# RoyAPTX4869/RaLD

Measured on AMD Instinct MI355X. Metric: denoising steps/sec (whole node), higher is better.
Workload: dtype bf16

## Files before the change

### rald_amd/csrc/gemm.hip

```cpp
#include <algorithm>
#include <cstdlib>
#include <type_traits>

#include "common.h"
#include "kernels.h"
#include "gemm_epilogue.h"
#include "gemm_tile.h"

namespace rald {

template <int MT, int NT, int EPI>
__device__ __forceinline__ void gemm_epilogue(f32x4 (&acc)[MT][NT], const GemmArgs& a, int mb, int nb, int64_t coff, int fr, int fq) {
    if constexpr (EPI == EPI_GEGLU) {
        bf16* C = reinterpret_cast<bf16*>(a.C) + coff;
#pragma unroll
        for (int i = 0; i < MT; ++i) {
            const int m = mb + i * 16 + fr;
            if (m >= a.M) continue;
#pragma unroll
            for (int p = 0; p < NT / 2; ++p) {
                const int nx = nb + 32 * p + 4 * fq;
                const int ng = nx + 16;
                float4 bx = *reinterpret_cast<const float4*>(a.bias + nx);
                float4 bg = *reinterpret_cast<const float4*>(a.bias + ng);
                f32x4 x = acc[i][2 * p], g = acc[i][2 * p + 1];
                bf16x4 o = pack4((x[0] + bx.x) * gelu_erf(g[0] + bg.x), (x[1] + bx.y) * gelu_erf(g[1] + bg.y),
                                 (x[2] + bx.z) * gelu_erf(g[2] + bg.z), (x[3] + bx.w) * gelu_erf(g[3] + bg.w));
                const int c = nb / 2 + 16 * p + 4 * fq;
                *reinterpret_cast<bf16x4*>(C + (int64_t)m * a.ldc + c) = o;
            }
        }
    } else {
#pragma unroll
        for (int i = 0; i < MT; ++i) {
            const int m = mb + i * 16 + fr;
            if (m >= a.M) continue;
#pragma unroll
            for (int j = 0; j < NT; ++j) {
                const int n = nb + j * 16 + 4 * fq;
                if (n >= a.N) continue;
                f32x4 v = acc[i][j];
                float4 b = make_float4(0.f, 0.f, 0.f, 0.f);
                if (a.bias) b = *reinterpret_cast<const float4*>(a.bias + n);
                const float al = n < a.alpha_ncols ? a.alpha : 1.0f;
                if constexpr (EPI == EPI_BF16) {
                    bf16* C = reinterpret_cast<bf16*>(a.C) + coff;
                    *reinterpret_cast<bf16x4*>(C + (int64_t)m * a.ldc + n) =
                        pack4(al * v[0] + b.x, al * v[1] + b.y, al * v[2] + b.z, al * v[3] + b.w);
                } else if constexpr (EPI == EPI_F32) {
                    float* C = reinterpret_cast<float*>(a.C) + coff;
                    *reinterpret_cast<float4*>(C + (int64_t)m * a.ldc + n) =
                        make_float4(al * v[0] + b.x, al * v[1] + b.y, al * v[2] + b.z, al * v[3] + b.w);
                } else {
                    float* C = reinterpret_cast<float*>(a.C) + coff;
                    float4* p = reinterpret_cast<float4*>(C + (int64_t)m * a.ldc + n);
                    float4 r = *p;
                    *p = make_float4(r.x + v[0] + b.x, r.y + v[1] + b.y, r.z + v[2] + b.z, r.w + v[3] + b.w);
                }
            }
        }
    }
}


template <int BM, int BN, int EPI>
__global__ __launch_bounds__(256) void gemm_nt_kernel(GemmArgs a) {
    constexpr int BK = 64;
    constexpr int MT = BM / 32;
    constexpr int NT = BN / 32;
    constexpr int PA = BM / 32;
    constexpr int PB = BN / 32;
    __shared__ __attribute__((aligned(16))) unsigned char smem[2 * (BM + BN) * BK * 2];
    bf16x8* sA = reinterpret_cast<bf16x8*>(smem);
    bf16x8* sB = reinterpret_cast<bf16x8*>(smem + 2 * BM * BK * 2);

    const int tid = threadIdx.x;
    const int lane = tid & 63;
    const int wave = tid >> 6;
    const int wm = wave >> 1, wn = wave & 1;
    const int m0 = blockIdx.y * BM, n0 = blockIdx.x * BN;
    int64_t oa, ob, coff;
    gemm_batch_offsets(a, blockIdx.z, oa, ob, coff);
    const bf16* A = a.A + oa;
    const bf16* B = a.B + ob;

    const int srow = tid >> 3, schunk = tid & 7;
    const bf16* gA[PA];
    const bf16* gB[PB];
#pragma unroll
    for (int p = 0; p < PA; ++p) {
        int r = m0 + srow + 32 * p;
        r = r < a.M ? r : a.M - 1;
        gA[p] = A + (int64_t)r * a.lda + schunk * 8;
    }
#pragma unroll
    for (int p = 0; p < PB; ++p) {
        int r = n0 + srow + 32 * p;
        r = r < a.N ? r : a.N - 1;
        gB[p] = B + (int64_t)r * a.ldb + schunk * 8;
    }
    bf16x8 rA[PA], rB[PB];
    auto load_tile = [&](int kt) {
#pragma unroll
        for (int p = 0; p < PA; ++p) rA[p] = *reinterpret_cast<const bf16x8*>(gA[p] + kt * BK);
#pragma unroll
        for (int p = 0; p < PB; ++p) rB[p] = *reinterpret_cast<const bf16x8*>(gB[p] + kt * BK);
    };
    auto store_tile = [&](int buf) {
#pragma unroll
        for (int p = 0; p < PA; ++p) {
            int r = srow + 32 * p;
            sA[(buf * BM + r) * 8 + RALD_SWZ(r, schunk)] = rA[p];
        }
#pragma unroll
        for (int p = 0; p < PB; ++p) {
            int r = srow + 32 * p;
            sB[(buf * BN + r) * 8 + RALD_SWZ(r, schunk)] = rB[p];
        }
    };

    f32x4 acc[MT][NT];
#pragma unroll
    for (int i = 0; i < MT; ++i)
#pragma unroll
        for (int j = 0; j < NT; ++j) acc[i][j] = f32x4{0.f, 0.f, 0.f, 0.f};

    const int nk = a.K / BK;
    load_tile(0);
    store_tile(0);
    __syncthreads();
    const int fr = lane & 15, fq = lane >> 4;
    for (int kt = 0; kt < nk; ++kt) {
        const int buf = kt & 1;
        if (kt + 1 < nk) load_tile(kt + 1);
#pragma unroll
        for (int kk = 0; kk < 2; ++kk) {
            bf16x8 fa[MT], fb[NT];
            const int chunk = kk * 4 + fq;
#pragma unroll
            for (int i = 0; i < MT; ++i) {
                int r = wm * (BM / 2) + i * 16 + fr;
                fa[i] = sA[(buf * BM + r) * 8 + RALD_SWZ(r, chunk)];
            }
#pragma unroll
            for (int j = 0; j < NT; ++j) {
                int r = wn * (BN / 2) + j * 16 + fr;
                fb[j] = sB[(buf * BN + r) * 8 + RALD_SWZ(r, chunk)];
            }
#pragma unroll
            for (int i = 0; i < MT; ++i)
#pragma unroll
                for (int j = 0; j < NT; ++j)
                    acc[i][j] = __builtin_amdgcn_mfma_f32_16x16x32_bf16(fb[j], fa[i], acc[i][j], 0, 0, 0);
        }
        if (kt + 1 < nk) store_tile(buf ^ 1);
        __syncthreads();
    }
    gemm_epilogue<MT, NT, EPI>(acc, a, m0 + wm * (BM / 2), n0 + wn * (BN / 2), coff, fr, fq);
}

template <int BM, int BN, int WM, int WN, int NSTAGE, int EPI>
__global__ __launch_bounds__(WM * WN * 64) void gemm_nt_glds_kernel(GemmArgs a) {
    constexpr int BK = 64;
    constexpr int WAVES = WM * WN;
    constexpr int MT = BM / (16 * WM);
    constexpr int NT = BN / (16 * WN);
    constexpr int CA = BM / 8 / WAVES;
    constexpr int CB = BN / 8 / WAVES;
    constexpr int STAGE_BYTES = (BM + BN) * BK * 2;
    extern __shared__ __attribute__((aligned(16))) unsigned char smem[];

    const int tid = threadIdx.x;
    const int lane = tid & 63;
    const int wave = __builtin_amdgcn_readfirstlane(tid >> 6);
    const int wm = wave / WN, wn = wave % WN;
    int tm, tn;
    xcd_strip_tile(tm, tn);
    const int ntn = gridDim.x, nt = ntn * gridDim.y;
    int bz = blockIdx.z;
    if (nt < 8 && (gridDim.z & 7) == 0) {
        const int g = (blockIdx.z * gridDim.y + blockIdx.y) * gridDim.x + blockIdx.x;
        const int slot = g >> 3;
        bz = (slot / nt) * 8 + (g & 7);
        const int tl = slot % nt;
        tm = tl / ntn;
        tn = tl % ntn;
    }
    const int m0 = tm * BM, n0 = tn * BN;
    int64_t oa, ob, coff;
    gemm_batch_offsets(a, bz, oa, ob, coff);
    const bf16* A = a.A + oa;
    const bf16* B = a.B + ob;

    const int nk = a.K / BK;
    const bf16* gA[CA];
    const bf16* gB[CB];
    dma_sources<WAVES>(gA, A, a.lda, m0, a.M, wave, lane);
    dma_sources<WAVES>(gB, B, a.ldb, n0, a.N, wave, lane);
    auto stage = [&](int kt, int buf) { dma_stage<BM, WAVES>(gA, gB, kt, nk, smem + buf * STAGE_BYTES, wave); };

    f32x4 acc[MT][NT];
#pragma unroll
    for (int i = 0; i < MT; ++i)
#pragma unroll
        for (int j = 0; j < NT; ++j) acc[i][j] = f32x4{0.f, 0.f, 0.f, 0.f};

    const int fr = lane & 15, fq = lane >> 4;
    auto read_frags = [&](int buf, int kk, bf16x8 (&fa)[MT], bf16x8 (&fb)[NT]) {
        const bf16x8* sA = reinterpret_cast<const bf16x8*>(smem + buf * STAGE_BYTES);
        const bf16x8* sB = sA + BM * 8;
        const int chunk = kk * 4 + fq;
#pragma unroll
        for (int i = 0; i < MT; ++i) {
            const int r = wm * (BM / WM) + i * 16 + fr;
            fa[i] = sA[r * 8 + RALD_SWZ(r, chunk)];
        }
#pragma unroll
        for (int j = 0; j < NT; ++j) {
            const int r = wn * (BN / WN) + j * 16 + fr;
            fb[j] = sB[r * 8 + RALD_SWZ(r, chunk)];
        }
    };
    auto mfma_all = [&](const bf16x8 (&fa)[MT], const bf16x8 (&fb)[NT]) {
#pragma unroll
        for (int i = 0; i < MT; ++i)
#pragma unroll
            for (int j = 0; j < NT; ++j)
                acc[i][j] = __builtin_amdgcn_mfma_f32_16x16x32_bf16(fb[j], fa[i], acc[i][j], 0, 0, 0);
    };
    if constexpr (NSTAGE == 2) {
        bf16x8 fa0[MT], fb0[NT], fa1[MT], fb1[NT];
        constexpr int W_ALL = 0x0070;
        constexpr int W_ST1 = ((CA + CB) & 15) | (((CA + CB) >> 4) << 14) | 0x0f70;
        stage(0, 0);
        if (nk > 1) { stage(1, 1); __builtin_amdgcn_s_waitcnt(W_ST1); }
        else __builtin_amdgcn_s_waitcnt(W_ALL);
        __builtin_amdgcn_s_barrier();
        read_frags(0, 0, fa0, fb0);
        read_frags(0, 1, fa1, fb1);
        mfma_all(fa0, fb0);
        __builtin_amdgcn_s_waitcnt(W_ALL);
        __builtin_amdgcn_s_barrier();
        auto body = [&](int kt, auto with_dma) {
            const int cur = kt & 1;
            if constexpr (decltype(with_dma)::value) stage(kt + 1, cur ^ 1);
            read_frags(cur, 0, fa0, fb0);
            mfma_all(fa1, fb1);
            if constexpr (MT + NT == 12 && MT * NT == 32) {
                if constexpr (decltype(with_dma)::value) {
#pragma unroll
                    for (int g = 0; g < CA + CB; ++g) {
                        __builtin_amdgcn_sched_group_barrier(0x008, 1, 0);
                        __builtin_amdgcn_sched_group_barrier(0x010, 1, 0);
                    }
#pragma unroll
                    for (int g = 0; g < 12; ++g) {
                        __builtin_amdgcn_sched_group_barrier(0x008, 2, 0);
                        __builtin_amdgcn_sched_group_barrier(0x100, 1, 0);
                    }
                } else {
#pragma unroll
                    for (int g = 0; g < 12; ++g) {
                        __builtin_amdgcn_sched_group_barrier(0x008, 2, 0);
                        __builtin_amdgcn_sched_group_barrier(0x100, 1, 0);
                    }
                    __builtin_amdgcn_sched_group_barrier(0x008, 8, 0);
                }
            }
            __builtin_amdgcn_sched_barrier(0);
            read_frags(cur, 1, fa1, fb1);
            mfma_all(fa0, fb0);
            if constexpr (MT + NT == 12 && MT * NT == 32) {
#pragma unroll
                for (int g = 0; g < 12; ++g) {
                    __builtin_amdgcn_sched_group_barrier(0x008, 2, 0);
                    __builtin_amdgcn_sched_group_barrier(0x100, 1, 0);
                }
                __builtin_amdgcn_sched_group_barrier(0x008, 8, 0);
            }
            __builtin_amdgcn_sched_barrier(0);
            __builtin_amdgcn_s_waitcnt(W_ALL);
            __builtin_amdgcn_s_barrier();
        };
        for (int kt = 1; kt + 1 < nk; ++kt) body(kt, std::true_type{});
        if (nk > 1) body(nk - 1, std::false_type{});
        mfma_all(fa1, fb1);
    } else {
#pragma unroll
        for (int s = 0; s < NSTAGE - 1; ++s)
            if (s < nk) stage(s, s);
        for (int kt = 0; kt < nk; ++kt) {
            if (kt + NSTAGE - 2 < nk) asm volatile("s_waitcnt vmcnt(%0)" ::"n"((NSTAGE - 2) * (CA + CB)) : "memory");
            else asm volatile("s_waitcnt vmcnt(0)" ::: "memory");
            asm volatile("" ::: "memory");
            __builtin_amdgcn_s_barrier();
            asm volatile("" ::: "memory");
            if (kt + NSTAGE - 1 < nk) stage(kt + NSTAGE - 1, (kt + NSTAGE - 1) % NSTAGE);
#pragma unroll
            for (int kk = 0; kk < 2; ++kk) {
                bf16x8 fa[MT], fb[NT];
                read_frags(kt % NSTAGE, kk, fa, fb);
                mfma_all(fa, fb);
            }
        }
    }
    if constexpr (NSTAGE != 2) {
        asm volatile("" ::: "memory");
        __builtin_amdgcn_s_barrier();
        asm volatile("" ::: "memory");
    }
    gemm_epilogue_lds<MT, NT, EPI>(acc, a, m0 + wm * (BM / WM), n0 + wn * (BN / WN), coff, lane, smem + wave * EPI_PATCH_BYTES,
                                   reinterpret_cast<float*>(smem + WAVES * EPI_PATCH_BYTES) + wave * NT * 16);
}

constexpr int PERSIST_LDS_BYTES = 160 * 1024;
__device__ __forceinline__ void batched_tile_at(int g, int ntn, int ntm, int nbatch, int& bz, int& tm, int& tn) {
    const int nt = ntn * ntm;
    if (nt < 8 && (nbatch & 7) == 0) {
        const int slot = g >> 3;
        bz = (slot / nt) * 8 + (g & 7);
        const int tl = slot % nt;
        tm = tl / ntn;
        tn = tl % ntn;
    } else {
        bz = g / nt;
        xcd_strip_tile_at(g - bz * nt, ntn, ntm, tm, tn);
    }
}
template <int EPI>
__global__ __launch_bounds__(512) void gemm_nt_persist_kernel(GemmArgs a) {
    static_assert(EPI == EPI_BF16 || EPI == EPI_GEGLU || EPI == EPI_SOFTMAX64, "the persistent engine is built for the three bf16-output epilogues");
    constexpr bool BATCHED = EPI == EPI_SOFTMAX64, BIAS = EPI != EPI_SOFTMAX64;
    constexpr int BM = 256, BN = 256, BK = 64, WN = 2, MT = 4, NT = 8;
    constexpr int DW = 4;
    constexpr int CP = BM / 8 / DW;
    constexpr int STAGE_BYTES = (BM + BN) * BK * 2;
    constexpr int OC = (EPI == EPI_GEGLU) ? NT * 8 : NT * 16;
    constexpr int ROWB = OC * 2, STRIDE = ROWB + 16, LPR = ROWB / 16;
    constexpr int PR = (EPI == EPI_GEGLU) ? 16 : 8;
    constexpr int PATCH = PR * STRIDE;
    constexpr int NSLOT = 12;
    constexpr int RPI = 64 / LPR;
    constexpr int BIAS_OFF = 2 * STAGE_BYTES + 31 * 1024;
    static_assert(2 * STAGE_BYTES + NSLOT * PATCH <= BIAS_OFF && BIAS_OFF + BN * 4 <= PERSIST_LDS_BYTES && PR % RPI == 0 && (MT * 16 / PR) % 2 == 0,
                  "LDS plan; an even number of steps per tile keeps the slot parity across tiles");
    extern __shared__ __attribute__((aligned(16))) unsigned char smem[];
    float* tbias = reinterpret_cast<float*>(smem + BIAS_OFF);

    const int tid = threadIdx.x;
    const int lane = tid & 63;
    const int wave = __builtin_amdgcn_readfirstlane(tid >> 6);
    const int wm = wave / WN, wn = wave % WN;
    const bool dma = wave < DW;
    const int ntm = a.M / BM, ntn = a.N / BN, nt = ntm * ntn * (BATCHED ? a.batch : 1);
    const int nk = a.K / BK;
    const int fr = lane & 15, fq = lane >> 4;

    const unsigned voA = (unsigned)((lane >> 3) * (int)a.lda + RALD_SWZ(lane >> 3, lane & 7) * 8) * 2u;
    const unsigned voB = (unsigned)((lane >> 3) * (int)a.ldb + RALD_SWZ(lane >> 3, lane & 7) * 8) * 2u;
    const unsigned lds0 = (unsigned)(uintptr_t)(lds_void*)smem;
    auto dma_piece = [&](const char* base, unsigned voff, unsigned lds) {
        asm volatile("s_nop 0\n\tglobal_load_lds_dwordx4 %0, %1" ::"v"(voff), "s"(base), "{m0}"(lds) : "memory");
    };
    struct Tile { int64_t oa, ob, oc; int m0, n0; };
    auto tile_at = [&](int t) {
        int bz = 0, tm, tn;
        if constexpr (BATCHED) batched_tile_at(t, ntn, ntm, a.batch, bz, tm, tn);
        else xcd_strip_tile_at(t, ntn, ntm, tm, tn);
        return Tile{bz * a.strideA, bz * a.strideB, bz * a.strideC, tm * BM, tn * BN};
    };
    auto stage = [&](const Tile& T, int kt, int buf) {
        const char* pa = reinterpret_cast<const char*>(a.A) + (T.oa + (int64_t)(T.m0 + 8 * wave) * a.lda + kt * BK) * 2;
        const char* pb = reinterpret_cast<const char*>(a.B) + (T.ob + (int64_t)(T.n0 + 8 * wave) * a.ldb + kt * BK) * 2;
        const unsigned s = lds0 + buf * STAGE_BYTES + wave * 1024;
#pragma unroll
        for (int p = 0; p < CP; ++p) dma_piece(pa + (int64_t)p * (8 * DW * 2) * a.lda, voA, s + p * DW * 1024);
#pragma unroll
        for (int p = 0; p < CP; ++p) dma_piece(pb + (int64_t)p * (8 * DW * 2) * a.ldb, voB, s + BM * 128 + p * DW * 1024);
    };
    auto read_frags = [&](int buf, int kk, bf16x8 (&fa)[MT], bf16x8 (&fb)[NT]) {
        const bf16x8* sA = reinterpret_cast<const bf16x8*>(smem + buf * STAGE_BYTES);
        const bf16x8* sB = sA + BM * 8;
        const int chunk = kk * 4 + fq;
#pragma unroll
        for (int i = 0; i < MT; ++i) {
            const int r = wm * (MT * 16) + i * 16 + fr;
            fa[i] = sA[r * 8 + RALD_SWZ(r, chunk)];
        }
#pragma unroll
        for (int j = 0; j < NT; ++j) {
            const int r = wn * (NT * 16) + j * 16 + fr;
            fb[j] = sB[r * 8 + RALD_SWZ(r, chunk)];
        }
    };
    f32x4 acc[MT][NT];
    auto mfma_all = [&](const bf16x8 (&fa)[MT], const bf16x8 (&fb)[NT]) {
#pragma unroll
        for (int i = 0; i < MT; ++i)
#pragma unroll
            for (int j = 0; j < NT; ++j)
                acc[i][j] = __builtin_amdgcn_mfma_f32_16x16x32_bf16(fb[j], fa[i], acc[i][j], 0, 0, 0);
    };
    constexpr int W_ALL = 0x0070;
    constexpr int W_LGKM = 0xc07f;
    constexpr int W_ST1 = ((2 * CP) & 15) | (((2 * CP) >> 4) << 14) | 0x0070;
    auto hand_over = [&]() {
        if (dma) __builtin_amdgcn_s_waitcnt(W_ALL);
        else __builtin_amdgcn_s_waitcnt(W_LGKM);
        __builtin_amdgcn_s_barrier();
    };
    bf16x8 fa0[MT], fb0[NT], fa1[MT], fb1[NT];
    auto body = [&](const Tile& T, int kt, bool with_dma) {
        const int cur = kt & 1;
        if (with_dma && dma) stage(T, kt + 1, cur ^ 1);
        __builtin_amdgcn_sched_barrier(0);
        read_frags(cur, 0, fa0, fb0);
        mfma_all(fa1, fb1);
#pragma unroll
        for (int g = 0; g < 12; ++g) {
            __builtin_amdgcn_sched_group_barrier(0x008, 2, 0);
            __builtin_amdgcn_sched_group_barrier(0x100, 1, 0);
        }
        __builtin_amdgcn_sched_group_barrier(0x008, 8, 0);
        __builtin_amdgcn_sched_barrier(0);
        read_frags(cur, 1, fa1, fb1);
        mfma_all(fa0, fb0);
#pragma unroll
        for (int g = 0; g < 12; ++g) {
            __builtin_amdgcn_sched_group_barrier(0x008, 2, 0);
            __builtin_amdgcn_sched_group_barrier(0x100, 1, 0);
        }
        __builtin_amdgcn_sched_group_barrier(0x008, 8, 0);
        __builtin_amdgcn_sched_barrier(0);
        hand_over();
    };

    if constexpr (BIAS)
        if (!a.bias && tid < BN / 4) *reinterpret_cast<float4*>(tbias + 4 * tid) = make_float4(0.f, 0.f, 0.f, 0.f);
    int t = blockIdx.x;
    Tile T = tile_at(t);
    if (dma) {
        stage(T, 0, 0);
        if (nk > 1) stage(T, 1, 1);
    }
    for (;;) {
#pragma unroll
        for (int i = 0; i < MT; ++i)
#pragma unroll
            for (int j = 0; j < NT; ++j) acc[i][j] = f32x4{0.f, 0.f, 0.f, 0.f};
        if (dma) {
            if (nk > 1) __builtin_amdgcn_s_waitcnt(W_ST1);
            else __builtin_amdgcn_s_waitcnt(W_ALL);
        } else __builtin_amdgcn_s_waitcnt(W_LGKM);
        __builtin_amdgcn_s_barrier();
        if constexpr (BIAS)
            if (wave == 0 && a.bias) dma_piece(reinterpret_cast<const char*>(a.bias + T.n0), 16u * lane, lds0 + BIAS_OFF);
        read_frags(0, 0, fa0, fb0);
        read_frags(0, 1, fa1, fb1);
        mfma_all(fa0, fb0);
        hand_over();
        for (int kt = 1; kt + 1 < nk; ++kt) body(T, kt, true);
        if (nk > 1) body(T, nk - 1, false);
        const int tnext = t + gridDim.x;
        Tile Tn = T;
        if (tnext < nt) {
            Tn = tile_at(tnext);
            if (dma) {
                stage(Tn, 0, 0);
                if (nk > 1) stage(Tn, 1, 1);
            }
        }
        mfma_all(fa1, fb1);

        {
            int lane_e = lane;
            asm volatile("" : "+v"(lane_e));
            const int fr = lane_e & 15, fq = lane_e >> 4;
            unsigned char* slot0 = smem + 2 * STAGE_BYTES + wave * PATCH;
            unsigned char* slot1 = slot0 + (dma ? 8 * PATCH : 0);
            const int mb = T.m0 + wm * (MT * 16), nb = T.n0 + wn * (NT * 16);
            const int oc0 = (EPI == EPI_GEGLU) ? nb / 2 : nb;
            const float* wbias = tbias + wn * (NT * 16);
            bf16* C = reinterpret_cast<bf16*>(a.C) + T.oc;
#pragma unroll
            for (int i = 0; i < MT; ++i) {
                bf16x4 sm[EPI == EPI_SOFTMAX64 ? NT : 1];
                if constexpr (EPI == EPI_SOFTMAX64) {
#pragma unroll
                    for (int g = 0; g < NT / 4; ++g) {
                        float e[16];
                        float mx = -3.0e38f;
#pragma unroll
                        for (int q = 0; q < 4; ++q)
#pragma unroll
                            for (int c = 0; c < 4; ++c) { e[4 * q + c] = a.alpha * acc[i][4 * g + q][c]; mx = fmaxf(mx, e[4 * q + c]); }
                        mx = fmaxf(mx, __shfl_xor(mx, 16, 64));
                        mx = fmaxf(mx, __shfl_xor(mx, 32, 64));
                        float su = 0.f;
#pragma unroll
                        for (int q = 0; q < 16; ++q) { e[q] = __builtin_amdgcn_exp2f(e[q] - mx); su += e[q]; }
                        su += __shfl_xor(su, 16, 64);
                        su += __shfl_xor(su, 32, 64);
                        const float inv = 1.0f / su;
#pragma unroll
                        for (int q = 0; q < 4; ++q) sm[4 * g + q] = pack4(e[4 * q] * inv, e[4 * q + 1] * inv, e[4 * q + 2] * inv, e[4 * q + 3] * inv);
                    }
                }
#pragma unroll
                for (int h = 0; h < 16 / PR; ++h) {
                    const int odd = (i * (16 / PR) + h) & 1;
                    unsigned char* patch = odd ? slot1 : slot0;
                    asm volatile("" ::: "memory");
                    if (PR == 16 || (fr >> 3) == h) {
                        const int pr = fr & (PR - 1);
                        if constexpr (EPI == EPI_GEGLU) {
#pragma unroll
                            for (int p = 0; p < NT / 2; ++p) {
                                const float4 bx = *reinterpret_cast<const float4*>(wbias + 32 * p + 4 * fq);
                                const float4 bg = *reinterpret_cast<const float4*>(wbias + 32 * p + 4 * fq + 16);
                                const f32x4 x = acc[i][2 * p], g = acc[i][2 * p + 1];
                                const f32x2 g01 = gelu_poly2(f32x2{g[0] + bg.x, g[1] + bg.y});
                                const f32x2 g23 = gelu_poly2(f32x2{g[2] + bg.z, g[3] + bg.w});
                                const f32x2 o01 = f32x2{x[0] + bx.x, x[1] + bx.y} * g01;
                                const f32x2 o23 = f32x2{x[2] + bx.z, x[3] + bx.w} * g23;
                                *reinterpret_cast<bf16x4*>(patch + pr * STRIDE + (16 * p + 4 * fq) * 2) = pack4(o01[0], o01[1], o23[0], o23[1]);
                            }
                        } else if constexpr (EPI == EPI_SOFTMAX64) {
#pragma unroll
                            for (int j = 0; j < NT; ++j) *reinterpret_cast<bf16x4*>(patch + pr * STRIDE + (16 * j + 4 * fq) * 2) = sm[j];
                        } else {
#pragma unroll
                            for (int j = 0; j < NT; ++j) {
                                const int n = nb + j * 16 + 4 * fq;
                                const float4 b = *reinterpret_cast<const float4*>(wbias + 16 * j + 4 * fq);
                                const f32x4 v = acc[i][j];
                                const float al = n < a.alpha_ncols ? a.alpha : 1.0f;
                                const float o0 = al * v[0] + b.x, o1 = al * v[1] + b.y, o2 = al * v[2] + b.z, o3 = al * v[3] + b.w;
                                *reinterpret_cast<bf16x4*>(patch + pr * STRIDE + (16 * j + 4 * fq) * 2) = pack4(o0, o1, o2, o3);
                            }
                        }
                    }
                    asm volatile("" ::: "memory");
                    __builtin_amdgcn_s_waitcnt(W_LGKM);
                    asm volatile("" ::: "memory");
                    const int r = lane_e / LPR, pc = lane_e % LPR;
                    uint4 v[2][PR / RPI];
                    if (!dma) {
#pragma unroll
                        for (int q = 0; q < PR / RPI; ++q) v[0][q] = *reinterpret_cast<const uint4*>(slot0 + (q * RPI + r) * STRIDE + pc * 16);
                    }
                    asm volatile("" ::: "memory");
                    __builtin_amdgcn_s_barrier();
                    asm volatile("" ::: "memory");
                    if (!dma) {
                        const unsigned char* partner = slot0 - DW * PATCH + (odd ? 8 * PATCH : 0);
#pragma unroll
                        for (int q = 0; q < PR / RPI; ++q) v[1][q] = *reinterpret_cast<const uint4*>(partner + (q * RPI + r) * STRIDE + pc * 16);
#pragma unroll
                        for (int w2 = 0; w2 < 2; ++w2)
#pragma unroll
                            for (int q = 0; q < PR / RPI; ++q) {
                                const int m = mb - w2 * (BM / 2) + i * 16 + h * PR + q * RPI + r;
                                bf16* Cp = C + (int64_t)m * a.ldc + oc0 + pc * 8;
                                typedef unsigned int u32x4 __attribute__((ext_vector_type(4)));
                                const u32x4 vv = u32x4{v[w2][q].x, v[w2][q].y, v[w2][q].z, v[w2][q].w};
                                asm volatile("global_store_dwordx4 %0, %1, off sc0 sc1 nt\n\ts_nop 1" ::"v"(Cp), "v"(vv) : "memory");
                            }
                    }
                    asm volatile("" ::: "memory");
                }
            }
        }
        if (tnext >= nt) break;
        t = tnext;
        T = Tn;
    }
}

template <int BM, int BN>
static int launch_tile(const GemmArgs& a, int epi, hipStream_t st) {
    dim3 grid(cdiv(a.N, BN), cdiv(a.M, BM), a.batch * a.batch2);
    switch (epi) {
        case EPI_BF16:  hipLaunchKernelGGL((gemm_nt_kernel<BM, BN, EPI_BF16>), grid, dim3(256), 0, st, a); break;
        case EPI_F32:   hipLaunchKernelGGL((gemm_nt_kernel<BM, BN, EPI_F32>), grid, dim3(256), 0, st, a); break;
        case EPI_RESID: hipLaunchKernelGGL((gemm_nt_kernel<BM, BN, EPI_RESID>), grid, dim3(256), 0, st, a); break;
        case EPI_GEGLU: hipLaunchKernelGGL((gemm_nt_kernel<BM, BN, EPI_GEGLU>), grid, dim3(256), 0, st, a); break;
        default: set_error("gemm: bad epilogue"); return 1;
    }
    RALD_HIP(hipGetLastError());
    return 0;
}

template <int BM, int BN, int WM, int WN, int NSTAGE, int EPI>
static int launch_glds_epi(const GemmArgs& a, hipStream_t st) {
    constexpr int WAVES = WM * WN;
    constexpr int smem = NSTAGE * (BM + BN) * 64 * 2;
    static_assert(smem >= epi_lds_bytes<BN / (16 * WN)>(WAVES), "epilogue patches and bias slots must fit in the staging buffers");
    static bool raised = false;
    return launch_dyn_lds(gemm_nt_glds_kernel<BM, BN, WM, WN, NSTAGE, EPI>, raised, dim3(cdiv(a.N, BN), cdiv(a.M, BM), a.batch * a.batch2), WAVES * 64, smem, st, a);
}
template <int BM, int BN, int WM, int WN, int NSTAGE>
static int launch_glds(const GemmArgs& a, int epi, hipStream_t st) {
    switch (epi) {
        case EPI_BF16:  return launch_glds_epi<BM, BN, WM, WN, NSTAGE, EPI_BF16>(a, st);
        case EPI_F32:   return launch_glds_epi<BM, BN, WM, WN, NSTAGE, EPI_F32>(a, st);
        case EPI_RESID: return launch_glds_epi<BM, BN, WM, WN, NSTAGE, EPI_RESID>(a, st);
        case EPI_GEGLU: return launch_glds_epi<BM, BN, WM, WN, NSTAGE, EPI_GEGLU>(a, st);
        case EPI_F16S:
            if constexpr ((BM == 64 && BN == 64) || (BM == 128 && BN == 128 && NSTAGE == 2)) return launch_glds_epi<BM, BN, WM, WN, NSTAGE, EPI_F16S>(a, st);
            else { set_error("gemm: the fp16-slab epilogue is built for the 64x64 ring and the 128x128 LDS-DMA engines"); return 1; }
        case EPI_SOFTMAX64:
            if constexpr ((BN / WN) % 64 == 0 && BM >= 128) return launch_glds_epi<BM, BN, WM, WN, NSTAGE, EPI_SOFTMAX64>(a, st);
            else { set_error("gemm: the softmax epilogue needs waves of 64-column groups"); return 1; }
        default: set_error("gemm: bad epilogue"); return 1;
    }
}

static int cu_count(int& cus) {
    static int cached[64] = {};
    int dev = 0;
    RALD_HIP(hipGetDevice(&dev));
    RALD_CHECK(dev >= 0 && dev < 64, "gemm: device index out of range");
    if (cached[dev] == 0) RALD_HIP(hipDeviceGetAttribute(&cached[dev], hipDeviceAttributeMultiprocessorCount, dev));
    cus = cached[dev];
    return 0;
}
static int launch_persist(const GemmArgs& a, int epi, int max_workgroups, hipStream_t st) {
    int cus = 0;
    if (int rc = cu_count(cus)) return rc;
    const int64_t tiles = (int64_t)(a.M / 256) * (a.N / 256) * a.batch;
    RALD_CHECK(tiles < (1ll << 30), "gemm: too many tiles for the persistent engine's tile index");
    const int grid = (int)std::min<int64_t>(tiles, std::min(cus, max_workgroups));
    RALD_CHECK(grid >= 1, "gemm: the persistent engine needs at least one workgroup");
    static bool raised_bf16 = false, raised_geglu = false, raised_softmax = false;
    switch (epi) {
        case EPI_SOFTMAX64: return launch_dyn_lds(gemm_nt_persist_kernel<EPI_SOFTMAX64>, raised_softmax, dim3(grid), 512, PERSIST_LDS_BYTES, st, a);
        case EPI_BF16:  return launch_dyn_lds(gemm_nt_persist_kernel<EPI_BF16>, raised_bf16, dim3(grid), 512, PERSIST_LDS_BYTES, st, a);
        case EPI_GEGLU: return launch_dyn_lds(gemm_nt_persist_kernel<EPI_GEGLU>, raised_geglu, dim3(grid), 512, PERSIST_LDS_BYTES, st, a);
        default: set_error("gemm: the persistent engine has the bf16, GEGLU and softmax epilogues"); return 1;
    }
}

int f16_saturation_gemm(unsigned* count, bool reset) {
    RALD_HIP(hipMemcpyFromSymbol(count, HIP_SYMBOL(g_f16_sat_gemm), sizeof(unsigned)));
    if (reset) { const unsigned z = 0; RALD_HIP(hipMemcpyToSymbol(HIP_SYMBOL(g_f16_sat_gemm), &z, sizeof(unsigned))); }
    return 0;
}

int gemm_nt(const GemmArgs& a0, int epi, hipStream_t st) {
    GemmArgs a = a0;
    a.flags |= GEMM_NT_STORE;
    RALD_CHECK(a.M > 0 && a.N > 0 && a.K > 0 && a.batch > 0 && a.batch2 > 0, "gemm: empty problem");
    const int64_t nbatch = (int64_t)a.batch * a.batch2;
    RALD_CHECK(nbatch <= 65535, "gemm: batch * batch2 exceeds the grid z limit");
    RALD_CHECK(a.K % 64 == 0, "gemm: K must be a multiple of 64 (pad with zeros)");
    RALD_CHECK(a.N % 4 == 0, "gemm: N must be a multiple of 4");
    RALD_CHECK(a.lda % 8 == 0 && a.ldb % 8 == 0, "gemm: lda/ldb must be multiples of 8 elements (16-byte rows)");
    RALD_CHECK(a.lda >= a.K && a.ldb >= a.K, "gemm: leading dimension smaller than K");
    RALD_CHECK(((uintptr_t)a.A % 16 == 0) && ((uintptr_t)a.B % 16 == 0) && ((uintptr_t)a.C % 16 == 0), "gemm: pointers must be 16-byte aligned");
    RALD_CHECK(a.ldc % 4 == 0, "gemm: ldc must be a multiple of 4");
    if (epi == EPI_GEGLU) {
        RALD_CHECK(a.N % 128 == 0 && a.bias != nullptr, "gemm: GEGLU needs N % 128 == 0 and a packed bias");
        RALD_CHECK(a.ldc >= a.N / 2, "gemm: GEGLU ldc < N/2");
    } else {
        RALD_CHECK(a.ldc >= a.N, "gemm: ldc < N");
    }
    if (epi == EPI_F16S) {
        RALD_CHECK(!a.out8 && a.N % 8 == 0, "gemm: the fp16-slab epilogue needs N % 8 == 0");
        const int64_t w128 = (int64_t)cdiv(a.M, 128) * cdiv(a.N, 128) * nbatch, w64 = (int64_t)cdiv(a.M, 64) * cdiv(a.N, 64) * nbatch;
        RALD_CHECK(w128 >= 192 || w64 <= 256, "gemm: fp16 slabs are not built for the register-staged engine (ask gemm_f16s_ok first)");
        if (w128 >= 192) return launch_glds<128, 128, 2, 2, 2>(a, epi, st);
        return launch_glds<64, 64, 2, 2, 8>(a, epi, st);
    }
    if (epi == EPI_SOFTMAX64) {
        RALD_CHECK(a.M % 128 == 0 && a.N % 128 == 0 && !a.bias && !a.out8 && a.alpha_ncols >= a.N, "gemm: the softmax epilogue needs M, N % 128 == 0 and no bias");
        if (a.M % 256 == 0 && a.N % 256 == 0) {
            const int64_t wg256 = (int64_t)(a.M / 256) * (a.N / 256) * nbatch;
            if (a.batch2 == 1) {
                int cus = 0;
                if (int rc = cu_count(cus)) return rc;
                if (wg256 >= 2 * (int64_t)cus) return launch_persist(a, epi, 1 << 30, st);
            }
            if (wg256 >= 256) return launch_glds<256, 256, 4, 2, 2>(a, epi, st);
        }
        return launch_glds<128, 128, 2, 2, 2>(a, epi, st);
    }
    if (a.out8) {
        RALD_CHECK(epi == EPI_GEGLU && a.outs && a.batch * a.batch2 == 1 && a.M % 256 == 0 && a.N % 256 == 0 && (a.N / 2) % 32 == 0 &&
                   (int64_t)(a.M / 256) * (a.N / 256) >= 256, "gemm: the MXFP8 output form needs the GEGLU epilogue on full 256x256 tiles");
        return launch_glds<256, 256, 4, 2, 2>(a, epi, st);
    }
    const int64_t wg128 = (int64_t)cdiv(a.M, 128) * cdiv(a.N, 128) * nbatch;
    if (wg128 < 192) {
        const int64_t wg64 = (int64_t)cdiv(a.M, 64) * cdiv(a.N, 64) * nbatch;
        if (wg64 > 256) return launch_tile<64, 64>(a, epi, st);
        return launch_glds<64, 64, 2, 2, 8>(a, epi, st);
    }
    const int64_t wg256 = (int64_t)(a.M / 256) * (a.N / 256) * nbatch;
    if (a.M % 256 == 0 && a.N % 256 == 0 && wg256 >= 256) {
        if (nbatch == 1 && (epi == EPI_BF16 || epi == EPI_GEGLU)) {
            int cus = 0;
            if (int rc = cu_count(cus)) return rc;
            if (wg256 >= 2 * (int64_t)cus) return launch_persist(a, epi, 1 << 30, st);
        }
        return launch_glds<256, 256, 4, 2, 2>(a, epi, st);
    }
    if (epi != EPI_GEGLU && wg128 <= 320 && a.M % 64 == 0) return launch_glds<64, 128, 2, 2, 3>(a, epi, st);
    return launch_glds<128, 128, 2, 2, 2>(a, epi, st);
}

int gemm_nt_256_test(const GemmArgs& a0, int epi, int persistent, int max_workgroups, hipStream_t st) {
    GemmArgs a = a0;
    a.flags |= GEMM_NT_STORE;
    RALD_CHECK(epi == EPI_BF16 || epi == EPI_GEGLU, "gemm_nt_256_test: EPI_BF16 or EPI_GEGLU");
    RALD_CHECK(a.M > 0 && a.N > 0 && a.K > 0 && a.M % 256 == 0 && a.N % 256 == 0 && a.K % 64 == 0, "gemm_nt_256_test: M, N % 256 == 0 and K % 64 == 0");
    RALD_CHECK(a.batch == 1 && a.batch2 == 1 && !a.out8, "gemm_nt_256_test: one problem, bf16 output");
    RALD_CHECK(a.lda % 8 == 0 && a.ldb % 8 == 0 && a.lda >= a.K && a.ldb >= a.K, "gemm_nt_256_test: lda/ldb must be multiples of 8 and at least K");
    RALD_CHECK(((uintptr_t)a.A % 16 == 0) && ((uintptr_t)a.B % 16 == 0) && ((uintptr_t)a.C % 16 == 0) && ((uintptr_t)a.bias % 16 == 0),
               "gemm_nt_256_test: pointers must be 16-byte aligned");
    RALD_CHECK(a.ldc % 8 == 0 && a.ldc >= (epi == EPI_GEGLU ? a.N / 2 : a.N), "gemm_nt_256_test: ldc");
    RALD_CHECK(epi != EPI_GEGLU || a.bias, "gemm_nt_256_test: GEGLU needs a packed bias");
    RALD_CHECK(max_workgroups >= 1, "gemm_nt_256_test: max_workgroups must be at least 1");
    if (persistent) return launch_persist(a, epi, max_workgroups, st);
    return launch_glds<256, 256, 4, 2, 2>(a, epi, st);
}

int gemm_nt_256_batched_test(const GemmArgs& a0, int epi, int persistent, int max_workgroups, hipStream_t st) {
    GemmArgs a = a0;
    a.flags |= GEMM_NT_STORE;
    RALD_CHECK(epi == EPI_BF16 || epi == EPI_GEGLU || epi == EPI_SOFTMAX64, "gemm_nt_256_batched_test: EPI_BF16, EPI_GEGLU or EPI_SOFTMAX64");
    RALD_CHECK(a.M > 0 && a.N > 0 && a.K > 0 && a.M % 256 == 0 && a.N % 256 == 0 && a.K % 64 == 0,
               "gemm_nt_256_batched_test: M, N % 256 == 0 and K % 64 == 0 (full tiles only)");
    RALD_CHECK(a.batch >= 1 && a.batch <= 65535 && !a.out8, "gemm_nt_256_batched_test: 1 <= batch <= 65535, bf16 output");
    RALD_CHECK(a.batch2 == 1, "gemm_nt_256_batched_test: batch2 must be 1 (the engine has no inner batch)");
    RALD_CHECK(a.lda % 8 == 0 && a.ldb % 8 == 0 && a.lda >= a.K && a.ldb >= a.K, "gemm_nt_256_batched_test: lda/ldb must be multiples of 8 and at least K");
    RALD_CHECK(((uintptr_t)a.A % 16 == 0) && ((uintptr_t)a.B % 16 == 0) && ((uintptr_t)a.C % 16 == 0) && ((uintptr_t)a.bias % 16 == 0),
               "gemm_nt_256_batched_test: pointers must be 16-byte aligned");
    const int ncols = epi == EPI_GEGLU ? a.N / 2 : a.N;
    RALD_CHECK(a.ldc % 8 == 0 && a.ldc >= ncols, "gemm_nt_256_batched_test: ldc");
    RALD_CHECK(a.strideA >= 0 && a.strideB >= 0 && a.strideA % 8 == 0 && a.strideB % 8 == 0 && a.strideC % 8 == 0,
               "gemm_nt_256_batched_test: strides must be non-negative multiples of 8 elements");
    RALD_CHECK(a.batch == 1 || a.strideC >= (int64_t)(a.M - 1) * a.ldc + ncols, "gemm_nt_256_batched_test: strideC lets the outputs of two entries overlap");
    RALD_CHECK(epi != EPI_GEGLU || a.bias, "gemm_nt_256_batched_test: GEGLU needs a packed bias");
    RALD_CHECK(epi != EPI_SOFTMAX64 || (!a.bias && a.alpha_ncols >= a.N), "gemm_nt_256_batched_test: the softmax epilogue takes no bias and one alpha");
    RALD_CHECK(max_workgroups >= 1, "gemm_nt_256_batched_test: max_workgroups must be at least 1");
    RALD_CHECK(!persistent || a.batch == 1 || epi == EPI_SOFTMAX64, "gemm_nt_256_batched_test: the persistent engine is batched for EPI_SOFTMAX64 only");
    if (persistent) return launch_persist(a, epi, max_workgroups, st);
    return launch_glds<256, 256, 4, 2, 2>(a, epi, st);
}

}
```

Baseline: 5923.

## Add drain epilogue for final persistent tile and widen persistent softmax dispatch

On a block's last tile, the persistent GEMM now uses a simpler epilogue. Each wave stages its own 16-row patch in the now-idle stage buffer 0 and stores directly, with no slot-parity handoff between DMA and compute waves. The shared epilogue code is factored into softmax/patch/store helpers. The softmax GEMM dispatch now picks the persistent kernel once the tile count reaches the CU count, rather than twice the CU count, so more shapes run on it, some of which may have a less balanced tail.

```diff
diff --git a/rald_amd/csrc/gemm.hip b/rald_amd/csrc/gemm.hip
--- a/rald_amd/csrc/gemm.hip
+++ b/rald_amd/csrc/gemm.hip
@@ -344,6 +344,7 @@
     constexpr int BIAS_OFF = 2 * STAGE_BYTES + 31 * 1024;
     static_assert(2 * STAGE_BYTES + NSLOT * PATCH <= BIAS_OFF && BIAS_OFF + BN * 4 <= PERSIST_LDS_BYTES && PR % RPI == 0 && (MT * 16 / PR) % 2 == 0,
                   "LDS plan; an even number of steps per tile keeps the slot parity across tiles");
+    static_assert(8 * 16 * STRIDE <= STAGE_BYTES && 16 % RPI == 0, "drain epilogue: eight wave-private 16-row patches in stage buffer 0");
     extern __shared__ __attribute__((aligned(16))) unsigned char smem[];
     float* tbias = reinterpret_cast<float*>(smem + BIAS_OFF);
 
@@ -433,6 +434,62 @@
         __builtin_amdgcn_sched_group_barrier(0x008, 8, 0);
         __builtin_amdgcn_sched_barrier(0);
         hand_over();
+    };
+    auto softmax_tile = [&](int i, bf16x4 (&sm)[EPI == EPI_SOFTMAX64 ? NT : 1]) {
+        if constexpr (EPI == EPI_SOFTMAX64) {
+#pragma unroll
+            for (int g = 0; g < NT / 4; ++g) {
+                float e[16];
+                float mx = -3.0e38f;
+#pragma unroll
+                for (int q = 0; q < 4; ++q)
+#pragma unroll
+                    for (int c = 0; c < 4; ++c) { e[4 * q + c] = a.alpha * acc[i][4 * g + q][c]; mx = fmaxf(mx, e[4 * q + c]); }
+                mx = fmaxf(mx, __shfl_xor(mx, 16, 64));
+                mx = fmaxf(mx, __shfl_xor(mx, 32, 64));
+                float su = 0.f;
+#pragma unroll
+                for (int q = 0; q < 16; ++q) { e[q] = __builtin_amdgcn_exp2f(e[q] - mx); su += e[q]; }
+                su += __shfl_xor(su, 16, 64);
+                su += __shfl_xor(su, 32, 64);
+                const float inv = 1.0f / su;
+#pragma unroll
+                for (int q = 0; q < 4; ++q) sm[4 * g + q] = pack4(e[4 * q] * inv, e[4 * q + 1] * inv, e[4 * q + 2] * inv, e[4 * q + 3] * inv);
+            }
+        }
+    };
+    auto patch_row = [&](int i, unsigned char* row, int fq, const float* wbias, int nb, const bf16x4 (&sm)[EPI == EPI_SOFTMAX64 ? NT : 1]) {
+        if constexpr (EPI == EPI_GEGLU) {
+#pragma unroll
+            for (int p = 0; p < NT / 2; ++p) {
+                const float4 bx = *reinterpret_cast<const float4*>(wbias + 32 * p + 4 * fq);
+                const float4 bg = *reinterpret_cast<const float4*>(wbias + 32 * p + 4 * fq + 16);
+                const f32x4 x = acc[i][2 * p], g = acc[i][2 * p + 1];
+                const f32x2 g01 = gelu_poly2(f32x2{g[0] + bg.x, g[1] + bg.y});
+                const f32x2 g23 = gelu_poly2(f32x2{g[2] + bg.z, g[3] + bg.w});
+                const f32x2 o01 = f32x2{x[0] + bx.x, x[1] + bx.y} * g01;
+                const f32x2 o23 = f32x2{x[2] + bx.z, x[3] + bx.w} * g23;
+                *reinterpret_cast<bf16x4*>(row + (16 * p + 4 * fq) * 2) = pack4(o01[0], o01[1], o23[0], o23[1]);
+            }
+        } else if constexpr (EPI == EPI_SOFTMAX64) {
+#pragma unroll
+            for (int j = 0; j < NT; ++j) *reinterpret_cast<bf16x4*>(row + (16 * j + 4 * fq) * 2) = sm[j];
+        } else {
+#pragma unroll
+            for (int j = 0; j < NT; ++j) {
+                const int n = nb + j * 16 + 4 * fq;
+                const float4 b = *reinterpret_cast<const float4*>(wbias + 16 * j + 4 * fq);
+                const f32x4 v = acc[i][j];
+                const float al = n < a.alpha_ncols ? a.alpha : 1.0f;
+                const float o0 = al * v[0] + b.x, o1 = al * v[1] + b.y, o2 = al * v[2] + b.z, o3 = al * v[3] + b.w;
+                *reinterpret_cast<bf16x4*>(row + (16 * j + 4 * fq) * 2) = pack4(o0, o1, o2, o3);
+            }
+        }
+    };
+    auto store_row = [](bf16* Cp, const uint4& v) {
+        typedef unsigned int u32x4 __attribute__((ext_vector_type(4)));
+        const u32x4 vv = u32x4{v.x, v.y, v.z, v.w};
+        asm volatile("global_store_dwordx4 %0, %1, off sc0 sc1 nt\n\ts_nop 1" ::"v"(Cp), "v"(vv) : "memory");
     };
 
     if constexpr (BIAS)
@@ -462,8 +519,9 @@
         for (int kt = 1; kt + 1 < nk; ++kt) body(T, kt, true);
         if (nk > 1) body(T, nk - 1, false);
         const int tnext = t + gridDim.x;
+        const bool last = tnext >= nt;
         Tile Tn = T;
-        if (tnext < nt) {
+        if (!last) {
             Tn = tile_at(tnext);
             if (dma) {
                 stage(Tn, 0, 0);
@@ -471,6 +529,36 @@
             }
         }
         mfma_all(fa1, fb1);
+
+        if (last) {
+            int lane_d = lane;
+            asm volatile("" : "+v"(lane_d));
+            const int fr = lane_d & 15, fq = lane_d >> 4;
+            unsigned char* patch = smem + wave * (16 * STRIDE);
+            const int mb = T.m0 + wm * (MT * 16), nb = T.n0 + wn * (NT * 16);
+            const int oc0 = (EPI == EPI_GEGLU) ? nb / 2 : nb;
+            const float* wbias = tbias + wn * (NT * 16);
+            const int r = lane_d / LPR, pc = lane_d % LPR;
+            bf16* Cp = reinterpret_cast<bf16*>(a.C) + T.oc + (int64_t)(mb + r) * a.ldc + oc0 + pc * 8;
+            const int64_t rstep = (int64_t)RPI * a.ldc;
+#pragma unroll
+            for (int i = 0; i < MT; ++i) {
+                bf16x4 sm[EPI == EPI_SOFTMAX64 ? NT : 1];
+                if constexpr (EPI == EPI_SOFTMAX64) softmax_tile(i, sm);
+                asm volatile("" ::: "memory");
+                patch_row(i, patch + fr * STRIDE, fq, wbias, nb, sm);
+                asm volatile("" ::: "memory");
+                uint4 v[16 / RPI];
+#pragma unroll
+                for (int q = 0; q < 16 / RPI; ++q) v[q] = *reinterpret_cast<const uint4*>(patch + (q * RPI + r) * STRIDE + pc * 16);
+#pragma unroll
+                for (int q = 0; q < 16 / RPI; ++q) {
+                    store_row(Cp, v[q]);
+                    Cp += rstep;
+                }
+            }
+            break;
+        }
 
         {
             int lane_e = lane;
@@ -485,66 +573,20 @@
 #pragma unroll
             for (int i = 0; i < MT; ++i) {
                 bf16x4 sm[EPI == EPI_SOFTMAX64 ? NT : 1];
-                if constexpr (EPI == EPI_SOFTMAX64) {
-#pragma unroll
-                    for (int g = 0; g < NT / 4; ++g) {
-                        float e[16];
-                        float mx = -3.0e38f;
-#pragma unroll
-                        for (int q = 0; q < 4; ++q)
-#pragma unroll
-                            for (int c = 0; c < 4; ++c) { e[4 * q + c] = a.alpha * acc[i][4 * g + q][c]; mx = fmaxf(mx, e[4 * q + c]); }
-                        mx = fmaxf(mx, __shfl_xor(mx, 16, 64));
-                        mx = fmaxf(mx, __shfl_xor(mx, 32, 64));
-                        float su = 0.f;
-#pragma unroll
-                        for (int q = 0; q < 16; ++q) { e[q] = __builtin_amdgcn_exp2f(e[q] - mx); su += e[q]; }
-                        su += __shfl_xor(su, 16, 64);
-                        su += __shfl_xor(su, 32, 64);
-                        const float inv = 1.0f / su;
-#pragma unroll
-                        for (int q = 0; q < 4; ++q) sm[4 * g + q] = pack4(e[4 * q] * inv, e[4 * q + 1] * inv, e[4 * q + 2] * inv, e[4 * q + 3] * inv);
-                    }
-                }
+                if constexpr (EPI == EPI_SOFTMAX64) softmax_tile(i, sm);
 #pragma unroll
                 for (int h = 0; h < 16 / PR; ++h) {
                     const int odd = (i * (16 / PR) + h) & 1;
                     unsigned char* patch = odd ? slot1 : slot0;
                     asm volatile("" ::: "memory");
-                    if (PR == 16 || (fr >> 3) == h) {
-                        const int pr = fr & (PR - 1);
-                        if constexpr (EPI == EPI_GEGLU) {
-#pragma unroll
-                            for (int p = 0; p < NT / 2; ++p) {
-                                const float4 bx = *reinterpret_cast<const float4*>(wbias + 32 * p + 4 * fq);
-                                const float4 bg = *reinterpret_cast<const float4*>(wbias + 32 * p + 4 * fq + 16);
-                                const f32x4 x = acc[i][2 * p], g = acc[i][2 * p + 1];
-                                const f32x2 g01 = gelu_poly2(f32x2{g[0] + bg.x, g[1] + bg.y});
-                                const f32x2 g23 = gelu_poly2(f32x2{g[2] + bg.z, g[3] + bg.w});
-                                const f32x2 o01 = f32x2{x[0] + bx.x, x[1] + bx.y} * g01;
-                                const f32x2 o23 = f32x2{x[2] + bx.z, x[3] + bx.w} * g23;
-                                *reinterpret_cast<bf16x4*>(patch + pr * STRIDE + (16 * p + 4 * fq) * 2) = pack4(o01[0], o01[1], o23[0], o23[1]);
-                            }
-                        } else if constexpr (EPI == EPI_SOFTMAX64) {
-#pragma unroll
-                            for (int j = 0; j < NT; ++j) *reinterpret_cast<bf16x4*>(patch + pr * STRIDE + (16 * j + 4 * fq) * 2) = sm[j];
-                        } else {
-#pragma unroll
-                            for (int j = 0; j < NT; ++j) {
-                                const int n = nb + j * 16 + 4 * fq;
-                                const float4 b = *reinterpret_cast<const float4*>(wbias + 16 * j + 4 * fq);
-                                const f32x4 v = acc[i][j];
-                                const float al = n < a.alpha_ncols ? a.alpha : 1.0f;
-                                const float o0 = al * v[0] + b.x, o1 = al * v[1] + b.y, o2 = al * v[2] + b.z, o3 = al * v[3] + b.w;
-                                *reinterpret_cast<bf16x4*>(patch + pr * STRIDE + (16 * j + 4 * fq) * 2) = pack4(o0, o1, o2, o3);
-                            }
-                        }
-                    }
+                    if (PR == 16 || (fr >> 3) == h) patch_row(i, patch + (fr & (PR - 1)) * STRIDE, fq, wbias, nb, sm);
                     asm volatile("" ::: "memory");
                     __builtin_amdgcn_s_waitcnt(W_LGKM);
                     asm volatile("" ::: "memory");
                     const int r = lane_e / LPR, pc = lane_e % LPR;
                     uint4 v[2][PR / RPI];
+#pragma unroll
+                    for (int q = 0; q < PR / RPI; ++q) asm volatile("" : "=v"(v[0][q].x), "=v"(v[0][q].y), "=v"(v[0][q].z), "=v"(v[0][q].w));
                     if (!dma) {
 #pragma unroll
                         for (int q = 0; q < PR / RPI; ++q) v[0][q] = *reinterpret_cast<const uint4*>(slot0 + (q * RPI + r) * STRIDE + pc * 16);
@@ -561,17 +603,13 @@
 #pragma unroll
                             for (int q = 0; q < PR / RPI; ++q) {
                                 const int m = mb - w2 * (BM / 2) + i * 16 + h * PR + q * RPI + r;
-                                bf16* Cp = C + (int64_t)m * a.ldc + oc0 + pc * 8;
-                                typedef unsigned int u32x4 __attribute__((ext_vector_type(4)));
-                                const u32x4 vv = u32x4{v[w2][q].x, v[w2][q].y, v[w2][q].z, v[w2][q].w};
-                                asm volatile("global_store_dwordx4 %0, %1, off sc0 sc1 nt\n\ts_nop 1" ::"v"(Cp), "v"(vv) : "memory");
+                                store_row(C + (int64_t)m * a.ldc + oc0 + pc * 8, v[w2][q]);
                             }
                     }
                     asm volatile("" ::: "memory");
                 }
             }
         }
-        if (tnext >= nt) break;
         t = tnext;
         T = Tn;
     }
@@ -679,7 +717,7 @@
             if (a.batch2 == 1) {
                 int cus = 0;
                 if (int rc = cu_count(cus)) return rc;
-                if (wg256 >= 2 * (int64_t)cus) return launch_persist(a, epi, 1 << 30, st);
+                if (wg256 >= (int64_t)cus) return launch_persist(a, epi, 1 << 30, st);
             }
             if (wg256 >= 256) return launch_glds<256, 256, 4, 2, 2>(a, epi, st);
         }
```

Measured after the change: 5938 (median of 4 runs). About the same (+0.3%).
